# mit-han-lab/TinyChatEngine

Measured on NVIDIA H100. Metric: llama3_8b_awq_int4_batch1_decode_tokens_per_s, higher is better.
Workload: dtype w4a16 (int4 weights; activations fp16 -> 32-bit block fixed point = four int8 digit planes; int32 accumulate, fp32 scale)

## Files before the change

tinychatengine_b200/csrc/decode_persistent.cu:

```cuda
#include <stdio.h>

#include "persistent.h"
#include "w4a16_act_planes.cuh"

namespace tce {
namespace pk {

namespace {

TCE_DEVINL unsigned ld_acquire_gpu(const unsigned *p) {
    unsigned v;
    asm volatile("ld.acquire.gpu.global.u32 %0, [%1];" : "=r"(v) : "l"(p) : "memory");
    return v;
}
TCE_DEVINL void red_release_gpu(unsigned *p) { asm volatile("red.release.gpu.global.add.u32 [%0], 1;" ::"l"(p) : "memory"); }

TCE_DEVINL void st_ll(uint2 *p, uint32_t data, uint32_t tag, bool sys) {
    if (sys)
        asm volatile("st.relaxed.sys.global.v2.b32 [%0], {%1, %2};" ::"l"(p), "r"(data), "r"(tag) : "memory");
    else
        asm volatile("st.relaxed.gpu.global.v2.b32 [%0], {%1, %2};" ::"l"(p), "r"(data), "r"(tag) : "memory");
}
TCE_DEVINL uint4 ld_ll2(const uint2 *p, bool sys) {
    uint4 r;
// ... 109 lines not shown
    float *gx;
    int *gsum;
    float *red;
    float *rms;
    float *inv;
    float *rope;
    uint64_t *full, *empty, *red_full, *red_empty;
    uint64_t *rx;
    float *prx;
    uint64_t *prx_full;
    uint64_t *pfree;
    int2 *red_pos;
    uint32_t ring_u32, xs_u32, gx_u32, gsum_u32, full_u32, empty_u32, redfull_u32, redempty_u32;
    int nst;
};

__host__ __device__ inline int resid_floats(const Args &a) { return plane_ic(a.E / kW4Group); }

TCE_DEVINL PSmem carve(uint8_t *raw, const Args &a) {
    PSmem s;
    uint8_t *base = raw + ((1024u - (smem_u32(raw) & 1023u)) & 1023u);
    s.nst = a.nst;
    s.ring = base;
    uint8_t *p = base + (size_t)a.nst * kStageBytes;
    s.xs = p;
    p += a.xs_bytes;
    s.resid = reinterpret_cast<float *>(p);
    p += (size_t)resid_floats(a) * 4;
    s.gx = reinterpret_cast<float *>(p);
    p += (size_t)a.max_ng * 4;
    s.gsum = reinterpret_cast<int *>(p);
    p += (size_t)a.max_ng * 8;
    s.red = reinterpret_cast<float *>(p);
    p += (size_t)kRedBufs * kCW * 16 * 4;
    s.rms = reinterpret_cast<float *>(p);
    p += 32 * 4;
    s.inv = reinterpret_cast<float *>(p);
    p += kCW * 4;
    s.rope = reinterpret_cast<float *>(p);
    p += 256 * 4;
    s.prx = reinterpret_cast<float *>(p);
    p += kPairSlots * 16 * 4;
    s.full = reinterpret_cast<uint64_t *>(p);
    s.empty = s.full + a.nst;
    s.red_full = s.empty + a.nst;
    s.red_empty = s.red_full + kRedBufs;
    s.rx = s.red_empty + kRedBufs;
    s.prx_full = s.rx + 1;
    s.pfree = s.prx_full + kPairSlots;
    s.red_pos = reinterpret_cast<int2 *>(s.pfree + kPairSlots);
    s.ring_u32 = smem_u32(s.ring);
    s.xs_u32 = smem_u32(s.xs);
    s.gx_u32 = smem_u32(s.gx);
    s.gsum_u32 = smem_u32(s.gsum);
    s.full_u32 = smem_u32(s.full);
    s.empty_u32 = smem_u32(s.empty);
    s.redfull_u32 = smem_u32(s.red_full);
    s.redempty_u32 = smem_u32(s.red_empty);
    return s;
}

struct Ring {
    int stage = 0;
    uint32_t phase = 0;
    TCE_DEVINL void advance(int nst) {
        if (++stage == nst) {
            stage = 0;
            phase ^= 1;
        }
    }
};
struct Red {
    int rb = 0;
    uint32_t rphase = 0;
    TCE_DEVINL void advance() {
// ... 11 lines not shown
    t0 = (int)((T * (unsigned)cta) / (unsigned)ncta);
    t1 = (int)((T * (unsigned)(cta + 1)) / (unsigned)ncta);
}

struct AttnSplit {
    int kvh, split, ch0, ch1, nsplit;
};
TCE_DEVINL AttnSplit attn_split(int cta, int ncta, int KVH, int pos) {
    AttnSplit s;
    const int T = pos + 1;
    const int nch = (T + kKvChunk - 1) / kKvChunk;
    int NS = ncta / KVH;
    if (NS < 1) NS = 1;
    int cps = (nch + NS - 1) / NS;
    if (cps * 32 < nch) cps = (nch + 31) / 32;
    s.nsplit = (nch + cps - 1) / cps;
    s.kvh = cta / NS;
    s.split = cta - s.kvh * NS;
    if (s.kvh >= KVH || s.split >= s.nsplit) {
        s.ch0 = s.ch1 = 0;
        s.kvh = 0;
    } else {
        s.ch0 = s.split * cps;
        s.ch1 = min(nch, s.ch0 + cps);
    }
    return s;
}

TCE_DEVINL void produce_gemv(const GemvOp &op, const CUtensorMap *m0, const uint8_t *meta, const PSmem &sm, Ring &rs, int cta, int ncta, int rank,
                             uint32_t leader, uint64_t policy) {
    int t0, t1;
    partition(op, cta, ncta, t0, t1);
    const KRange kr = k_range(op.NG, rank);
    const uint32_t box_bytes = 16u * (uint32_t)kr.bw * 64u;
    const int nbox = (t1 - t0) * kr.nb;
    const uint8_t *rec = meta + (size_t)t0 * kr.nb * kBoxMetaBytes;
    int tile = t0, box = 0;
    for (int i = 0; i < nbox; i += 2) {
        const int n = min(2, nbox - i);
        mbar_wait(&sm.empty[rs.stage], rs.phase ^ 1);
        uint64_t *bar = &sm.full[rs.stage];
        uint8_t *dst = sm.ring + (size_t)rs.stage * kStageBytes;
        mbar_arrive_expect_tx_pred(bar, (uint32_t)n * (box_bytes + kBoxMetaBytes), leader);
#pragma unroll 1
        for (int b = 0; b < n; b++) {
            int row = op.gate_up ? tile * 8 : tile * 16;
            const CUtensorMap *m = m0;
            if (!op.gate_up && op.nseg > 1 && row >= op.rows0) {
                row -= op.rows0;
                m = m0 + 1;
                if (op.nseg > 2 && row >= op.rows1) {
                    row -= op.rows1;
                    m = m0 + 2;
                }
            }
            tma_load_3d_pred(dst + b * 16384, m, 0, row, box * kBoxGroups, bar, policy, leader);
            if (op.gate_up) tma_load_3d_pred(dst + b * 16384 + 8192, m + 1, 0, row, box * kBoxGroups, bar, policy, leader);
            if (++box == kr.nb) {
                box = 0;
                tile++;
            }
        }
        bulk_g2s_pred(dst + kMetaOff, rec + (size_t)i * kBoxMetaBytes, (uint32_t)n * kBoxMetaBytes, bar, policy, leader);
        __syncwarp();
        rs.advance(sm.nst);
    }
}

TCE_DEVINL void produce_attn(const Args &a, const LayerDesc &L, const CUtensorMap *kvmap, const PSmem &sm, Ring &rs, int cta, int ncta, int pos,
                             uint32_t leader, uint64_t policy) {
    const AttnSplit sp = attn_split(cta, ncta, a.KVH, pos);
    for (int c = sp.ch0; c < sp.ch1; c++) {
        mbar_wait(&sm.empty[rs.stage], rs.phase ^ 1);
        uint64_t *bar = &sm.full[rs.stage];
        uint8_t *dst = sm.ring + (size_t)rs.stage * kStageBytes;
        const int krow = L.k_row0 + sp.kvh * a.max_ctx + c * kKvChunk, vrow = L.v_row0 + sp.kvh * a.max_ctx + c * kKvChunk;
        mbar_arrive_expect_tx_pred(bar, 2u * kHalfBytes, leader);
        tma_load_2d_pred(dst, kvmap, 0, krow, bar, policy, leader);
        tma_load_2d_pred(dst + 8192, kvmap, 64, krow, bar, policy, leader);
        tma_load_2d_pred(dst + kHalfBytes, kvmap, 0, vrow, bar, policy, leader);
        tma_load_2d_pred(dst + kHalfBytes + 8192, kvmap, 64, vrow, bar, policy, leader);
        __syncwarp();
        rs.advance(sm.nst);
    }
}

TCE_DEVINL void producer_walk(const Args &a, const PSmem &sm, int cta, int ncta, int rank, int pos, int lane) {
    Ring rs;
    const uint64_t policy = l2_policy_evict_first();
    const uint32_t leader = (lane == 0) ? 1u : 0u;
    const int Lyr = a.num_layers, nphase = 5 * Lyr + 1;
    const CUtensorMap *wmaps = a.maps + (size_t)rank * (Lyr * 7 + 1);
    const CUtensorMap *kvmap = a.maps + (size_t)2 * (Lyr * 7 + 1);
#pragma unroll 1
    for (int p = 0; p < nphase; p++) {
        const int l = p / 5, k = p - 5 * l;
// ... 169 lines not shown
                const float4 r1 = *reinterpret_cast<const float4 *>(sm.resid + (size_t)ui * 8 + 4);
                x[0] = r0.x; x[1] = r0.y; x[2] = r0.z; x[3] = r0.w;
                x[4] = r1.x; x[5] = r1.y; x[6] = r1.z; x[7] = r1.w;
                if (a.tp_size == 1) {
                    uint4 w[4];
                    wait_ll2xN<4>(delta + (size_t)gu * 8, tag, false, w);
                    x[0] += __uint_as_float(w[0].x); x[1] += __uint_as_float(w[0].z); x[2] += __uint_as_float(w[1].x); x[3] += __uint_as_float(w[1].z);
                    x[4] += __uint_as_float(w[2].x); x[5] += __uint_as_float(w[2].z); x[6] += __uint_as_float(w[3].x); x[7] += __uint_as_float(w[3].z);
                } else {
                    tp_accumulate(x, delta + (size_t)gu * 8, a.tp_size, a.E, tag);
                }
            }
            *reinterpret_cast<float4 *>(sm.resid + (size_t)ui * 8) = make_float4(x[0], x[1], x[2], x[3]);
            *reinterpret_cast<float4 *>(sm.resid + (size_t)ui * 8 + 4) = make_float4(x[4], x[5], x[6], x[7]);
        }
        if (emit) {
#pragma unroll
            for (int i = 0; i < 8; i++) ss += x[i] * x[i];
            v[0] = x[0] * g0.x; v[1] = x[1] * g0.y; v[2] = x[2] * g0.z; v[3] = x[3] * g0.w;
            v[4] = x[4] * g1.x; v[5] = x[5] * g1.y; v[6] = x[6] * g1.z; v[7] = x[7] * g1.w;
            gemv::emit_unit<1>(sm.xs, xic, sm.gx, sm.gsum, ui, valid, v, lane);
        }
    }
    if (!emit) return;
    ss = warp_sum(ss);
    if (lane == 0) {
        sm.rms[pc.rank * kCW + cw] = ss;
        st_async_b32(pc.r_rms + (uint32_t)(pc.rank * kCW + cw) * 4u, __float_as_uint(ss), pc.r_bar);
    }
    named_bar_sync(1, kConsumerThreads);
}

struct UnitRegs {
    uint4 wa, wb, xe, xo;
    uint32_t z;
    uint32_t sc;
    int sxv;
};
TCE_DEVINL void unit_compute(const UnitRegs &u, uint32_t st_addr, float lscale, float &totA, float &totB) {
    constexpr uint32_t ML = 0x0f0f0f0fu, MH = 0xf0f0f0f0u;
    int accL[4], accH[4];
    mma_m16n8k32_u8s8_z(accL, u.wa.x & ML, u.wb.x & ML, u.wa.y & ML, u.wb.y & ML, u.xe.x, u.xe.y);
    mma_m16n8k32_u8s8_z(accH, u.wa.x & MH, u.wb.x & MH, u.wa.y & MH, u.wb.y & MH, u.xo.x, u.xo.y);
    mma_m16n8k32_u8s8(accL, u.wa.z & ML, u.wb.z & ML, u.wa.w & ML, u.wb.w & ML, u.xe.z, u.xe.w);
    mma_m16n8k32_u8s8(accH, u.wa.z & MH, u.wb.z & MH, u.wa.w & MH, u.wb.w & MH, u.xo.z, u.xo.w);
    const float2 sc = h2_to_f2(u.sc);
    const float st = lds_f32(st_addr) * lscale;
    const int zAq = (int)(u.z & 0xFFu), zBq = (int)(u.z >> 8);
    const int vA = (accL[0] << 8) + accL[1] + (((accH[0] << 8) + accH[1]) >> 4) - zAq * u.sxv;
    const int vB = (accL[2] << 8) + accL[3] + (((accH[2] << 8) + accH[3]) >> 4) - zBq * u.sxv;
    totA += (sc.x * st) * (float)vA;
    totB += (sc.y * st) * (float)vB;
}

TCE_DEVINL void hand_tile(const Args &a, const GemvOp &op, const PSmem &sm, Red &cs, float totA, float totB, int cw, int lane) {
    const int g = lane >> 2, t = lane & 3;
    float inv = sm.inv[cw];
    if (inv < 0.f) {
        mbar_wait_u32(smem_u32(sm.rx), inv < -1.5f ? 1u : 0u);
        inv = rms_inv(sm, op.IC, a.eps);
        __syncwarp();
        if (lane == 0) sm.inv[cw] = inv;
    }
    totA += __shfl_xor_sync(0xffffffffu, totA, 1);
    totB += __shfl_xor_sync(0xffffffffu, totB, 1);
    mbar_wait_u32(sm.redempty_u32 + (uint32_t)cs.rb * 8u, cs.rphase ^ 1);
    float *rbuf = sm.red + ((size_t)cs.rb * kCW + cw) * 16;
    if (t == 0) {
        rbuf[g] = totA * inv;
        rbuf[g + 8] = totB * inv;
    }
    __syncwarp();
    if (lane == 0) mbar_arrive_u32(sm.redfull_u32 + (uint32_t)cs.rb * 8u);
    cs.advance();
}

TCE_DEVINL void consume_gemv(const Args &a, const GemvOp &op, const PSmem &sm, Ring &rs, int rx_parity, int cta, int ncta, int rank, int cw, int p, int nphase) {
    int lane;
    asm volatile("mov.u32 %0, %%laneid;" : "=r"(lane));
    if (lane == 0) sm.inv[cw] = rx_parity >= 0 ? -1.f - (float)rx_parity : 1.f;
    __syncwarp();
    Red cs;
    {
        const int2 rp = sm.red_pos[cw];
        cs.rb = rp.x;
        cs.rphase = (uint32_t)rp.y;
    }
    const int g = lane >> 2, t = lane & 3;
    int t0, t1;
    partition(op, cta, ncta, t0, t1);
    const KRange kr = k_range(op.NG, rank);
    const int nb = kr.nb, nbox = (t1 - t0) * nb;
    const int lim = kr.ng - cw;
    const uint32_t w_lane = (uint32_t)cw * (op.gate_up ? 512u : 1024u) + (uint32_t)g * 64u + (uint32_t)t * 16u;
    const uint32_t wb_off = op.gate_up ? 8192u : 512u;
    const uint32_t m_lane = (uint32_t)kMetaOff + (uint32_t)(cw * 8 + g) * 4u;
    const uint32_t z_lane = (uint32_t)kMetaOff + 512u + (uint32_t)(cw * 8 + g) * 2u;
    const uint32_t x_lane = sm.xs_u32 + (uint32_t)((g >> 1) & 1) * (uint32_t)plane_ic(op.NG) * 2u + (uint32_t)(t * 2 + (g & 1)) * 16u + (uint32_t)cw * 256u;
    const uint32_t s_lane = sm.gsum_u32 + (uint32_t)(2 * cw + (t & 1)) * 4u;
    const uint32_t q_lane = sm.gx_u32 + (uint32_t)cw * 4u;
    const float lscale = (t == 0) ? 65536.f : (t == 1 ? 1.f : 0.f);
    const bool xl = g < 4;
    if (a.dbg && nbox > 0 && cw == 0 && lane == 0) {
        mbar_wait_u32(sm.full_u32 + (uint32_t)rs.stage * 8u, rs.phase);
        stamp(a, cta, nphase, p, 4);
    }
    int box = 0;
    float totA = 0.f, totB = 0.f;
    for (int left = nbox; left > 0; left -= 2) {
        const int box0 = box, box1 = (box0 + 1 == nb) ? 0 : box0 + 1;
        const bool two = left > 1;
        box = (box1 + 1 == nb) ? 0 : box1 + 1;
        const bool has0 = box0 * kBoxGroups < lim, has1 = two && box1 * kBoxGroups < lim;
        mbar_wait_u32(sm.full_u32 + (uint32_t)rs.stage * 8u, rs.phase);
        const uint32_t base = sm.ring_u32 + (uint32_t)rs.stage * (uint32_t)kStageBytes;
        const uint32_t wb_ = base + w_lane, mb_ = base + m_lane, zb_ = base + z_lane;
        UnitRegs u0, u1;
        u0.xe = u0.xo = u1.xe = u1.xo = make_uint4(0u, 0u, 0u, 0u);
        if (has0) {
            const uint32_t xb_ = x_lane + (uint32_t)box0 * 4096u;
            u0.wa = lds_u4(wb_);
            u0.wb = lds_u4(wb_ + wb_off);
            if (xl) {
                u0.xe = lds_u4(xb_);
                u0.xo = lds_u4(xb_ + 128u);
            }
            u0.sc = lds_u32(mb_);
            u0.z = lds_u16(zb_);
            u0.sxv = (int)lds_u32(s_lane + (uint32_t)box0 * 128u);
        }
        if (has1) {
            const uint32_t xb_ = x_lane + (uint32_t)box1 * 4096u;
            u1.wa = lds_u4(wb_ + 16384u);
            u1.wb = lds_u4(wb_ + 16384u + wb_off);
            if (xl) {
                u1.xe = lds_u4(xb_);
                u1.xo = lds_u4(xb_ + 128u);
            }
            u1.sc = lds_u32(mb_ + (uint32_t)kBoxMetaBytes);
            u1.z = lds_u16(zb_ + (uint32_t)kBoxMetaBytes);
            u1.sxv = (int)lds_u32(s_lane + (uint32_t)box1 * 128u);
        }
        if (has0) unit_compute(u0, q_lane + (uint32_t)box0 * 64u, lscale, totA, totB);
        const bool end0 = box0 + 1 == nb;
        float hA = 0.f, hB = 0.f;
        if (end0) {
            hA = totA;
            hB = totB;
            totA = totB = 0.f;
        }
        if (has1) unit_compute(u1, q_lane + (uint32_t)box1 * 64u, lscale, totA, totB);
        __syncwarp();
        if (lane == 0) mbar_arrive_u32(sm.empty_u32 + (uint32_t)rs.stage * 8u);
        rs.advance(sm.nst);
        if (left <= 2 && cw == 0 && lane == 0) stamp(a, cta, nphase, p, 5);
        const bool end1 = two && box1 + 1 == nb;
        if (end0) hand_tile(a, op, sm, cs, hA, hB, cw, lane);
        if (end1) {
            hand_tile(a, op, sm, cs, totA, totB, cw, lane);
            totA = totB = 0.f;
        }
    }
    __syncwarp();
    if (lane == 0) sm.red_pos[cw] = make_int2(cs.rb, (int)cs.rphase);
    __syncwarp();
    if (cw == 0 && lane == 0) stamp(a, cta, nphase, p, 6);
}

struct EpiState {
    unsigned long long best;
    uint32_t nsent, nrecv;
};

TCE_DEVINL void epilogue_gemv(const Args &a, const GemvOp &op, const PSmem &sm, Red &es, EpiState &st, uint2 *out_ll, int which, uint32_t tag, int cta, int ncta,
                              int p, int nphase) {
    int lane;
    asm volatile("mov.u32 %0, %%laneid;" : "=r"(lane));
    int t0, t1;
    partition(op, cta, ncta, t0, t1);
    const bool tp = a.tp_size > 1;
    const uint32_t rank = cluster_rank();
    const int tsplit = t0 + (t1 - t0 + 1) / 2;
    for (int tile = t0; tile < t1; tile++) {
        mbar_wait_u32(sm.redfull_u32 + (uint32_t)es.rb * 8u, es.rphase);
        if (tile == t1 - 1 && lane == 0) stamp(a, cta, nphase, p, 7);
        const float *rbuf = sm.red + (size_t)es.rb * kCW * 16;
        float v = 0.f;
        {
            const int row = lane & 15, w0 = (lane >> 4) * 8;
#pragma unroll
            for (int w = 0; w < 8; w++) v += rbuf[(w0 + w) * 16 + row];
        }
        v += __shfl_down_sync(0xffffffffu, v, 16);
        __syncwarp();
        if (lane == 0) mbar_arrive_u32(sm.redempty_u32 + (uint32_t)es.rb * 8u);
        es.advance();
        const bool mine = (tile >= tsplit) == (rank == 1u);
        const uint32_t slot = (mine ? st.nrecv : st.nsent) % kPairSlots;
        if (!mine) {
            const uint32_t n = st.nsent++;
            mbar_wait_cluster(smem_u32(sm.pfree + slot), ((n / kPairSlots) & 1u) ^ 1u);
            if (lane < 16)
                st_async_b32(map_to_cta(smem_u32(sm.prx + slot * 16 + lane), rank ^ 1u), __float_as_uint(v), map_to_cta(smem_u32(sm.prx_full + slot), rank ^ 1u));
            continue;
        }
        const uint32_t n = st.nrecv++;
        const uint32_t fb = smem_u32(sm.prx_full + slot);
        if (lane == 0) asm volatile("mbarrier.arrive.expect_tx.shared::cta.b64 _, [%0], %1;" ::"r"(fb), "r"(64u) : "memory");
        mbar_wait_u32(fb, (n / kPairSlots) & 1u);
        v += sm.prx[slot * 16 + (lane & 15)];
        __syncwarp();
        if (lane == 0) mbar_arrive_remote(map_to_cta(smem_u32(sm.pfree + slot), rank ^ 1u));
        switch (op.epi) {
            case PE_DELTA_LL:
                if (lane < 16) {
                    const size_t o = (size_t)a.tp_rank * a.E + (size_t)tile * 16 + lane;
                    if (tp) {
                        for (int pr = 0; pr < a.tp_size; pr++) st_ll(a.tp_delta[which][pr] + o, __float_as_uint(v), tag, true);
                    } else {
                        st_ll(out_ll + o, __float_as_uint(v), tag, false);
                    }
                }
                break;
            case PE_HALF_LL: {
                const float hi = __shfl_down_sync(0xffffffffu, v, 1);
                if (lane < 16 && !(lane & 1)) st_ll(out_ll + (size_t)tile * 8 + (lane >> 1), pack_half2(v, hi), tag, false);
                break;
            }
            case PE_SILU_LL: {
                const float up = __shfl_down_sync(0xffffffffu, v, 8);
                const float y = v / (1.f + __expf(-v)) * up;
                const float yhi = __shfl_down_sync(0xffffffffu, y, 1);
                if (lane < 8 && !(lane & 1)) st_ll(out_ll + (size_t)tile * 4 + (lane >> 1), pack_half2(y, yhi), tag, false);
                break;
            }
            case PE_LOGITS:
                if (lane < 16) {
                    const int idx = tile * 16 + lane;
                    a.logits[idx] = v;
                    const unsigned long long key = argmax_key(v, a.vocab_base + idx);
                    st.best = key > st.best ? key : st.best;
                }
                break;
        }
    }
}

TCE_DEVINL uint32_t kv_off(int r, int c) { return (uint32_t)((c >> 3) * 8192 + r * 128 + (((c & 7) ^ (r & 7)) << 4)); }

TCE_DEVINL float2 rope_pair(const uint2 *vec, int j, uint32_t tag, const float *cosr, const float *sinr) {
    const uint2 *pa = vec + j, *pb = vec + (j < 32 ? j + 32 : j - 32);
    uint2 wa = ld_ll1(pa, false), wb = ld_ll1(pb, false);
    if (wa.y != tag) wa.x = wait_ll1(pa, tag, false);
    if (wb.y != tag) wb.x = wait_ll1(pb, tag, false);
    const float2 x = h2_to_f2(wa.x), xp = h2_to_f2(wb.x);
    const float sgn = (j < 32) ? -1.f : 1.f;
    const int d = 2 * j;
    return make_float2(x.x * cosr[d] + sgn * xp.x * sinr[d], x.y * cosr[d + 1] + sgn * xp.y * sinr[d + 1]);
}

TCE_DEVINL void attention_phase(const Args &a, const LayerDesc &L, const PSmem &sm, Ring &rs, uint32_t tag_qkv, uint32_t tag_part, uint32_t tag_out, int cta,
                                int ncta, int pos, int ctid, int cw, int lane, int p, int nphase) {
    const AttnSplit sp = attn_split(cta, ncta, a.KVH, pos);
    const int nrep = a.nrep;
    const int g = lane >> 2, t = lane & 3;
    if (sp.ch0 < sp.ch1) {
        __half *sQ = reinterpret_cast<__half *>(sm.xs);
        float *sO = reinterpret_cast<float *>(sm.xs + 8 * 136 * 2);
        float *sML = sO + (size_t)kCW * nrep * 128;
        uint32_t *sKV = reinterpret_cast<uint32_t *>(sML + (size_t)kCW * nrep * 2);
        const float *cosr = sm.rope, *sinr = sm.rope + 128;
        const bool owns_new = sp.ch1 * kKvChunk > pos;
        static_assert(8 * 64 == kConsumerThreads, "one pass");
        {
            const int r = ctid >> 6, j = ctid & 63;
            float2 v = make_float2(0.f, 0.f);
// ... 304 lines not shown
    if (cta == 0 && ctid == 0) {
        const unsigned target = (epoch + 1u) * (unsigned)ncta;
        const long long t0 = clock64();
        while ((int)(ld_acquire_gpu(a.done) - target) < 0) {
            if (clock64() - t0 > kSpinLimit) __trap();
        }
        unsigned long long key = *reinterpret_cast<volatile unsigned long long *>(a.argmax_cell);
        if (a.tp_size > 1) {
            const uint32_t tag = tag_base + 2u * (uint32_t)nphase;
            for (int pr = 0; pr < a.tp_size; pr++) {
                st_ll(a.tp_keys[pr] + (size_t)a.tp_rank * 2, (uint32_t)(key >> 32), tag, true);
                st_ll(a.tp_keys[pr] + (size_t)a.tp_rank * 2 + 1, (uint32_t)key, tag, true);
            }
            key = 0ull;
            for (int pr = 0; pr < a.tp_size; pr++) {
                const uint32_t hi = wait_ll1(a.tp_keys[a.tp_rank] + (size_t)pr * 2, tag, true), lo = wait_ll1(a.tp_keys[a.tp_rank] + (size_t)pr * 2 + 1, tag, true);
                const unsigned long long k2 = ((unsigned long long)hi << 32) | lo;
                key = k2 > key ? k2 : key;
            }
        }
        *a.next_token = (int)(0xFFFFFFFFu - (unsigned)(key & 0xFFFFFFFFull));
        *a.argmax_cell = 0ull;
        *a.epoch = epoch + 1u;
    }
}

__global__ void repack_meta_kernel(W4Seg s0, W4Seg s1, W4Seg s2, int nseg, int gate_up, int g0, int ng, int nb, int zeros_w, int sf_w, int num_tiles, uint8_t *out) {
    const int idx = blockIdx.x * blockDim.x + threadIdx.x;
    if (idx >= num_tiles * nb * kBoxGroups) return;
    const int gi = idx % kBoxGroups, rb = idx / kBoxGroups;
    const int tile = rb / nb, box = rb - tile * nb;
    const int lg = kBoxGroups * box + gi, G = g0 + lg;
    uint8_t *rec = out + (size_t)rb * kBoxMetaBytes;
    __half *so = reinterpret_cast<__half *>(rec) + gi * 16;
    uint8_t *zo = rec + 512 + gi * 16;
    for (int r = 0; r < 16; r++) {
        const W4Seg *seg = &s0;
        int row;
        if (gate_up) {
            seg = (r < 8) ? &s0 : &s1;
            row = tile * 8 + (r & 7);
        } else {
            row = tile * 16 + r;
            if (nseg > 1 && row >= s0.rows) {
                row -= s0.rows;
                seg = &s1;
                if (nseg > 2 && row >= s1.rows) {
                    row -= s1.rows;
                    seg = &s2;
                }
            }
        }
        const int slot = (r & 7) * 2 + (r >> 3);
        if (lg < ng) {
            so[slot] = seg->scales[(size_t)row * sf_w + G];
            zo[slot] = (uint8_t)((seg->zeros[(size_t)row * zeros_w + (G >> 3)] >> ((G & 7) * 4)) & 0xFu);
        } else {
            so[slot] = __float2half(0.f);
            zo[slot] = 0;
        }
    }
}

}

int attn_scratch_bytes(int nrep) { return 8 * 136 * 2 + kCW * nrep * 128 * 4 + kCW * nrep * 2 * 4 + 2 * 64 * 4; }

int attn_nsplit_max(int ncta, int KVH, int max_ctx) {
    int NS = ncta / KVH;
    if (NS < 1) NS = 1;
    const int nch = (max_ctx + kKvChunk - 1) / kKvChunk;
    return NS < nch ? NS : nch;
}

static size_t fixed_bytes(const Args &a) {
    return (size_t)a.xs_bytes + (size_t)resid_floats(a) * 4 + (size_t)a.max_ng * 12 + (size_t)kRedBufs * kCW * 16 * 4 + 32 * 4 + kCW * 4 + 256 * 4 + (size_t)kPairSlots * 16 * 4 +
           (size_t)(2 * kMaxStages + 2 * kRedBufs + 1 + 2 * kPairSlots) * 8 + (size_t)kCW * 8 + 1024;
}
void plan_smem(Args &a, int smem_optin) {
    int xs = attn_scratch_bytes(a.nrep);
    for (int i = 0; i < OPI_COUNT; i++) xs = max(xs, 4 * plane_ic(a.op[i].NG));
    a.xs_bytes = (xs + 15) & ~15;
    a.nst = 0;
    const long long n = ((long long)smem_optin - (long long)fixed_bytes(a)) / kStageBytes;
    if (n >= 2) a.nst = (int)(n > kMaxStages ? kMaxStages : n);
}
size_t smem_bytes(const Args &a) { return fixed_bytes(a) + (size_t)a.nst * kStageBytes; }

cudaError_t repack_meta(Ctx *ctx, const W4Seg *segs, int nseg, int gate_up, int IC, const KRange &kr, uint8_t *out, cudaStream_t stream) {
    int rows = 0;
    for (int i = 0; i < nseg; i++) rows += segs[i].rows;
    const int num_tiles = rows / 16;
    const int zw = zeros_width(IC, kW4Group);
    const int total = num_tiles * kr.nb * kBoxGroups;
    if (total == 0) return cudaSuccess;
    repack_meta_kernel<<<(total + 127) / 128, 128, 0, stream>>>(segs[0], segs[nseg > 1 ? 1 : 0], segs[nseg > 2 ? 2 : 0], nseg, gate_up, kr.g0, kr.ng, kr.nb, zw, zw * 8,
                                                               num_tiles, out);
    (void)ctx;
    return cudaGetLastError();
}

cudaError_t encode_kv_tmap(CUtensorMap *out, const void *kv, long long rows) {
    const TmapEncodeFn fn = tmap_encoder();
    if (!fn) return cudaErrorNotSupported;
    const cuuint64_t gdim[2] = {128, (cuuint64_t)rows};
    const cuuint64_t gstride[1] = {256};
    const cuuint32_t box[2] = {64, (cuuint32_t)kKvChunk};
    const cuuint32_t estr[2] = {1, 1};
    const CUresult r = fn(out, CU_TENSOR_MAP_DATA_TYPE_UINT16, 2, const_cast<void *>(kv), gdim, gstride, box, estr, CU_TENSOR_MAP_INTERLEAVE_NONE,
                          CU_TENSOR_MAP_SWIZZLE_128B, CU_TENSOR_MAP_L2_PROMOTION_L2_256B, CU_TENSOR_MAP_FLOAT_OOB_FILL_NONE);
    return r == CUDA_SUCCESS ? cudaSuccess : cudaErrorInvalidValue;
}

static cudaLaunchConfig_t launch_config(Ctx *ctx, size_t smem, cudaStream_t stream, cudaLaunchAttribute *attr) {
    cudaLaunchConfig_t cfg = {};
    cfg.gridDim = dim3(ctx->num_sms);
    cfg.blockDim = dim3(kThreads);
    cfg.dynamicSmemBytes = smem;
    cfg.stream = stream;
    attr[0].id = cudaLaunchAttributeClusterDimension;
    attr[0].val.clusterDim.x = 2;
    attr[0].val.clusterDim.y = 1;
    attr[0].val.clusterDim.z = 1;
    cfg.attrs = attr;
    cfg.numAttrs = 1;
// ... 28 lines not shown
```

tinychatengine_b200/csrc/llama_decoder.cu:

```cuda
#include "llama_decoder.h"

#include "persistent.h"

#include <math.h>
#include <stdio.h>
#include <stdlib.h>
#include <string.h>

namespace tce {

#define DCK(call)                              \
    do {                                       \
        cudaError_t e__ = (call);              \
        if (e__ != cudaSuccess) return e__;    \
    } while (0)

static bool w4_ok(const tce_w4_tensor &t, int oc, int ic) { return t.w && t.zeros && t.scales && t.oc == oc && t.ic == ic; }

LlamaDecoder *LlamaDecoder::create(Ctx *ctx, int attn_chunk, const tce_llama_config &cfg, const tce_llama_weights &w, std::string *err) {
    auto bad = [&](const char *m) {
        *err = m;
        return (LlamaDecoder *)nullptr;
    };
    if (cfg.head_dim != 128) return bad("head_dim must be 128");
// ... 106 lines not shown
    *count = (int)bs_->gemv_ops.size();
    return cudaSuccess;
}

cudaError_t LlamaDecoder::tp_handle(void *out64) {
    if (tp_ <= 1 || !tp_buf_) return cudaErrorInvalidValue;
    static_assert(sizeof(cudaIpcMemHandle_t) == 64, "handle size");
    return cudaIpcGetMemHandle(reinterpret_cast<cudaIpcMemHandle_t *>(out64), tp_buf_.get());
}

cudaError_t LlamaDecoder::tp_connect(const void *handles, std::string *err) {
    if (tp_ <= 1) return cudaErrorInvalidValue;
    const cudaIpcMemHandle_t *h = reinterpret_cast<const cudaIpcMemHandle_t *>(handles);
    for (int p = 0; p < tp_; p++) {
        if (p == cfg_.tp_rank) {
            tp_peer_[p] = tp_buf_.get();
        } else {
            DCK(cudaIpcOpenMemHandle((void **)&tp_peer_[p], h[p], cudaIpcMemLazyEnablePeerAccess));
        }
    }
    DCK(build_persistent(err));
    tp_connected_ = true;
    return cudaSuccess;
}

cudaError_t LlamaDecoder::build_persistent(std::string *err) {
    const int E = cfg_.embed_dim, F = cfg_.hidden_dim, H = cfg_.num_heads, KVH = cfg_.num_kv_heads, hd = cfg_.head_dim, V = cfg_.vocab_size;
    const int Lyr = cfg_.num_layers, ncta = ctx_->num_sms;
    const int nrep = H / KVH;
    auto no = [&](const char *m) {
        if (err) *err = m;
        return cudaErrorNotSupported;
    };
    if (hd != 128 || nrep > 4 || ncta < KVH || F % 16 || V % 16) return no("shape outside the persistent kernel's envelope");
    if (ncta % 2) return no("odd SM count: the persistent kernel runs on clusters of two CTAs");
    pk::Args a{};
    auto mk = [&](int IC, int rows, int nseg, int gate_up, int rows0, int rows1, int x_mode, int epi) {
        pk::GemvOp o{};
        o.IC = IC;
        o.NG = IC / kW4Group;
        o.num_tiles = rows / 16;
        o.nseg = nseg;
        o.gate_up = gate_up;
        o.rows0 = rows0;
        o.rows1 = rows1;
        o.x_mode = x_mode;
        o.epi = epi;
        return o;
    };
    const bool tp = tp_ > 1;
    a.op[pk::OPI_QKV] = mk(E, (H + 2 * KVH) * hd, 3, 0, H * hd, KVH * hd, pk::PX_RMS_F32, pk::PE_HALF_LL);
    a.op[pk::OPI_O] = mk(H * hd, E, 1, 0, E, 0, pk::PX_HALF, pk::PE_DELTA_LL);
    a.op[pk::OPI_GATEUP] = mk(E, 2 * F, 2, 1, F, F, pk::PX_RMS_F32, pk::PE_SILU_LL);
    a.op[pk::OPI_DOWN] = mk(F, E, 1, 0, E, 0, pk::PX_HALF, pk::PE_DELTA_LL);
    a.op[pk::OPI_LMHEAD] = mk(E, V, 1, 0, V, 0, pk::PX_RMS_F32, pk::PE_LOGITS);
    int max_ng = 0, min_ng = 1 << 30;
    for (int i = 0; i < pk::OPI_COUNT; i++) {
        if (a.op[i].NG > max_ng) max_ng = a.op[i].NG;
        if (a.op[i].NG < min_ng) min_ng = a.op[i].NG;
        if (a.op[i].IC % kW4Group || a.op[i].num_tiles < 1) return no("bad GEMV shape");
    }
    if (min_ng < 2) return no("a GEMV with a single 128-group: nothing to split across a cluster of two CTAs");
    a.max_ng = (max_ng + 3) & ~3;
    a.E = E;
    a.nrep = nrep;
    pk::plan_smem(a, ctx_->smem_optin);
    if (a.nst < 2) return no("shared memory too small for the persistent kernel");
    if (!pk::pair_supported(ctx_, a)) return no("the device cannot co-schedule num_sms / 2 clusters of two CTAs");

    auto dalloc = [&](size_t bytes) -> void * {
        DevPtr<uint8_t> p;
        if (dev_alloc(p, bytes ? bytes : 16) != cudaSuccess) return nullptr;
        pk_allocs_.push_back(std::move(p));
        return pk_allocs_.back().get();
    };
    cudaStream_t s = ctx_->stream;
    const size_t nmaps = (size_t)Lyr * 7 + 1;
    std::vector<CUtensorMap> maps(2 * nmaps + 1);
    memset(maps.data(), 0, maps.size() * sizeof(CUtensorMap));
    std::vector<pk::LayerDesc> descs(Lyr);
    const size_t per_kv = (size_t)KVH * cfg_.max_ctx;
    for (int l = 0; l < Lyr; l++) {
        const tce_llama_layer &L = layers_[l];
        const tce_w4_tensor *t7[7] = {&L.q, &L.k, &L.v, &L.o, &L.gate, &L.up, &L.down};
        const int opi[7] = {pk::OPI_QKV, pk::OPI_QKV, pk::OPI_QKV, pk::OPI_O, pk::OPI_GATEUP, pk::OPI_GATEUP, pk::OPI_DOWN};
        for (int rank = 0; rank < 2; rank++) {
            for (int i = 0; i < 7; i++) {
                const pk::GemvOp &o = a.op[opi[i]];
                const pk::KRange kr = pk::k_range(o.NG, rank);
                DCK(encode_w4_tmap_units(&maps[rank * nmaps + (size_t)l * 7 + i], t7[i]->w, t7[i]->oc, t7[i]->ic, kr.bw, o.gate_up ? 8 : 16, kr.g0, kr.ng));
            }
        }
        pk::LayerDesc &D = descs[l];
        memset(&D, 0, sizeof(D));
        const W4Seg qkv[3] = {seg_of(L.q), seg_of(L.k), seg_of(L.v)}, o1[1] = {seg_of(L.o)}, gu[2] = {seg_of(L.gate), seg_of(L.up)}, d1[1] = {seg_of(L.down)};
        const W4Seg *segs[4] = {qkv, o1, gu, d1};
        const int nsegs[4] = {3, 1, 2, 1};
        const int ops4[4] = {pk::OPI_QKV, pk::OPI_O, pk::OPI_GATEUP, pk::OPI_DOWN};
        for (int rank = 0; rank < 2; rank++) {
            for (int i = 0; i < 4; i++) {
                const pk::GemvOp &o = a.op[ops4[i]];
                const pk::KRange kr = pk::k_range(o.NG, rank);
                uint8_t *m = (uint8_t *)dalloc((size_t)o.num_tiles * kr.nb * pk::kBoxMetaBytes);
                if (!m) return cudaErrorMemoryAllocation;
                DCK(pk::repack_meta(ctx_, segs[i], nsegs[i], o.gate_up, o.IC, kr, m, s));
                D.meta[rank][i] = m;
            }
        }
        D.input_norm = L.input_norm;
        D.post_norm = L.post_norm;
        D.k_cache = (__half *)kv_cache(l, 0);
        D.v_cache = (__half *)kv_cache(l, 1);
        D.k_row0 = (int)(((size_t)l * 2 + 0) * per_kv);
        D.v_row0 = (int)(((size_t)l * 2 + 1) * per_kv);
    }
    {
        const pk::GemvOp &o = a.op[pk::OPI_LMHEAD];
        const W4Seg lm[1] = {seg_of(w_.lm_head)};
        for (int rank = 0; rank < 2; rank++) {
            const pk::KRange kr = pk::k_range(o.NG, rank);
            DCK(encode_w4_tmap_units(&maps[rank * nmaps + (size_t)Lyr * 7], w_.lm_head.w, w_.lm_head.oc, w_.lm_head.ic, kr.bw, 16, kr.g0, kr.ng));
            uint8_t *m = (uint8_t *)dalloc((size_t)o.num_tiles * kr.nb * pk::kBoxMetaBytes);
            if (!m) return cudaErrorMemoryAllocation;
            DCK(pk::repack_meta(ctx_, lm, 1, 0, o.IC, kr, m, s));
            a.lm_meta[rank] = m;
        }
    }
    DCK(pk::encode_kv_tmap(&maps[2 * nmaps], d_kv_.get(), (long long)Lyr * 2 * per_kv));
    CUtensorMap *dmaps = (CUtensorMap *)dalloc(maps.size() * sizeof(CUtensorMap));
    pk::LayerDesc *ddesc = (pk::LayerDesc *)dalloc(descs.size() * sizeof(pk::LayerDesc));
    a.nsplit_max = pk::attn_nsplit_max(ncta, KVH, cfg_.max_ctx);
    const size_t n_qkv = (size_t)(H + 2 * KVH) * 64, n_attn = (size_t)H * 64, n_act = (size_t)F / 2, n_part = (size_t)H * a.nsplit_max * 130;
    const size_t ll_words = n_qkv + n_attn + n_act + n_part + (tp ? 0 : (size_t)2 * E);
    uint2 *ll = (uint2 *)dalloc(ll_words * sizeof(uint2));
    uint8_t *ctl = (uint8_t *)dalloc(32);
    if (!dmaps || !ddesc || !ll || !ctl) return cudaErrorMemoryAllocation;
    DCK(cudaMemcpyAsync(dmaps, maps.data(), maps.size() * sizeof(CUtensorMap), cudaMemcpyHostToDevice, s));
    DCK(cudaMemcpyAsync(ddesc, descs.data(), descs.size() * sizeof(pk::LayerDesc), cudaMemcpyHostToDevice, s));
    DCK(cudaMemsetAsync(ll, 0, ll_words * sizeof(uint2), s));
    DCK(cudaMemsetAsync(ctl, 0, 32, s));
    DCK(cudaStreamSynchronize(s));
    a.layers = ddesc;
    a.num_layers = Lyr;
    a.maps = dmaps;
    a.final_norm = w_.final_norm;
    a.embed = (const __half *)w_.embed_f16;
    a.embed_rows = V * tp_;
    a.qkv_ll = ll;
    a.attn_ll = a.qkv_ll + n_qkv;
    a.act_ll = a.attn_ll + n_attn;
    a.part_ll = a.act_ll + n_act;
    a.logits = io1_.logits.get();
    a.tokpos = io1_.req.get();
    a.next_token = io1_.next.get();
// ... 888 lines not shown
```

tinychatengine_b200/csrc/persistent.h:

```cpp
#pragma once
#include "kernels.h"

namespace tce {
namespace pk {

constexpr int kCW = 16;
constexpr int kAuxWarps = 4;
constexpr int kThreads = 32 * (kAuxWarps + kCW);
constexpr int kConsumerThreads = 32 * kCW;
constexpr int kHalfBytes = 16384;
constexpr int kBoxGroups = 16;
constexpr int kMetaOff = 2 * kHalfBytes;
constexpr int kBoxMetaBytes = 768;
constexpr int kStageBytes = 34816;
constexpr int kMaxStages = 6;
constexpr int kRedBufs = 3;
constexpr int kPairSlots = 8;
constexpr int kKvChunk = 64;

enum XMode : int { PX_HALF = 0, PX_RMS_F32 = 1 };
enum Epi : int { PE_HALF_LL = 0, PE_DELTA_LL = 1, PE_SILU_LL = 2, PE_LOGITS = 3 };
enum OpIdx : int { OPI_QKV = 0, OPI_O = 1, OPI_GATEUP = 2, OPI_DOWN = 3, OPI_LMHEAD = 4, OPI_COUNT = 5 };

struct GemvOp {
    int IC, NG;
    int num_tiles;
    int nseg, gate_up;
    int rows0, rows1;
    int x_mode, epi;
};

struct KRange {
    int g0, ng;
    int nb, bw;
};
__host__ __device__ inline KRange k_range(int NG, int rank) {
    KRange k;
    const int h = (NG + 1) / 2;
    k.g0 = rank ? h : 0;
    k.ng = rank ? NG - h : h;
    k.nb = (k.ng + kBoxGroups - 1) / kBoxGroups;
    k.bw = k.ng < kBoxGroups ? k.ng : kBoxGroups;
    return k;
}
__host__ __device__ inline int plane_ic(int NG) { return k_range(NG, 0).ng * 128; }

// ... 55 lines not shown
```

Baseline: 515.4.

## Widen GEMV output tile from 16 to 32 rows per box

Doubles the rows per weight tile so each TMA box carries 32 output rows and one stage holds one box instead of two 16-row boxes. Each consumer warp now issues four MMA chains sharing the same activation fragments, which reuses activation loads across more rows and halves the per-tile reduction and handoff overhead. The metadata record layout, repack kernel, tensor-map box heights, reduction buffers and epilogues are all resized so every lane now owns one row. In exchange there are fewer tiles, so work balance across CTAs gets coarser for small matrices, and each warp holds more registers.

```diff
diff --git a/tinychatengine_b200/csrc/decode_persistent.cu b/tinychatengine_b200/csrc/decode_persistent.cu
--- a/tinychatengine_b200/csrc/decode_persistent.cu
+++ b/tinychatengine_b200/csrc/decode_persistent.cu
@@ -165,7 +165,7 @@
     s.gsum = reinterpret_cast<int *>(p);
     p += (size_t)a.max_ng * 8;
     s.red = reinterpret_cast<float *>(p);
-    p += (size_t)kRedBufs * kCW * 16 * 4;
+    p += (size_t)kRedBufs * kCW * kTileRows * 4;
     s.rms = reinterpret_cast<float *>(p);
     p += 32 * 4;
     s.inv = reinterpret_cast<float *>(p);
@@ -173,7 +173,7 @@
     s.rope = reinterpret_cast<float *>(p);
     p += 256 * 4;
     s.prx = reinterpret_cast<float *>(p);
-    p += kPairSlots * 16 * 4;
+    p += kPairSlots * kTileRows * 4;
     s.full = reinterpret_cast<uint64_t *>(p);
     s.empty = s.full + a.nst;
     s.red_full = s.empty + a.nst;
@@ -251,36 +251,32 @@
     int t0, t1;
     partition(op, cta, ncta, t0, t1);
     const KRange kr = k_range(op.NG, rank);
-    const uint32_t box_bytes = 16u * (uint32_t)kr.bw * 64u;
+    const uint32_t stage_tx = (uint32_t)kTileRows * (uint32_t)kr.bw * 64u + (uint32_t)kBoxMetaBytes;
     const int nbox = (t1 - t0) * kr.nb;
     const uint8_t *rec = meta + (size_t)t0 * kr.nb * kBoxMetaBytes;
     int tile = t0, box = 0;
-    for (int i = 0; i < nbox; i += 2) {
-        const int n = min(2, nbox - i);
+    for (int i = 0; i < nbox; i++) {
         mbar_wait(&sm.empty[rs.stage], rs.phase ^ 1);
         uint64_t *bar = &sm.full[rs.stage];
         uint8_t *dst = sm.ring + (size_t)rs.stage * kStageBytes;
-        mbar_arrive_expect_tx_pred(bar, (uint32_t)n * (box_bytes + kBoxMetaBytes), leader);
-#pragma unroll 1
-        for (int b = 0; b < n; b++) {
-            int row = op.gate_up ? tile * 8 : tile * 16;
-            const CUtensorMap *m = m0;
-            if (!op.gate_up && op.nseg > 1 && row >= op.rows0) {
-                row -= op.rows0;
-                m = m0 + 1;
-                if (op.nseg > 2 && row >= op.rows1) {
-                    row -= op.rows1;
-                    m = m0 + 2;
-                }
-            }
-            tma_load_3d_pred(dst + b * 16384, m, 0, row, box * kBoxGroups, bar, policy, leader);
-            if (op.gate_up) tma_load_3d_pred(dst + b * 16384 + 8192, m + 1, 0, row, box * kBoxGroups, bar, policy, leader);
-            if (++box == kr.nb) {
-                box = 0;
-                tile++;
-            }
-        }
-        bulk_g2s_pred(dst + kMetaOff, rec + (size_t)i * kBoxMetaBytes, (uint32_t)n * kBoxMetaBytes, bar, policy, leader);
+        mbar_arrive_expect_tx_pred(bar, stage_tx, leader);
+        int row = op.gate_up ? tile * (kTileRows / 2) : tile * kTileRows;
+        const CUtensorMap *m = m0;
+        if (!op.gate_up && op.nseg > 1 && row >= op.rows0) {
+            row -= op.rows0;
+            m = m0 + 1;
+            if (op.nseg > 2 && row >= op.rows1) {
+                row -= op.rows1;
+                m = m0 + 2;
+            }
+        }
+        tma_load_3d_pred(dst, m, 0, row, box * kBoxGroups, bar, policy, leader);
+        if (op.gate_up) tma_load_3d_pred(dst + 16384, m + 1, 0, row, box * kBoxGroups, bar, policy, leader);
+        bulk_g2s_pred(dst + kMetaOff, rec + (size_t)i * kBoxMetaBytes, (uint32_t)kBoxMetaBytes, bar, policy, leader);
+        if (++box == kr.nb) {
+            box = 0;
+            tile++;
+        }
         __syncwarp();
         rs.advance(sm.nst);
     }
@@ -516,28 +512,39 @@
 }
 
 struct UnitRegs {
-    uint4 wa, wb, xe, xo;
+    uint4 wa, wb, wc, wd, xe, xo;
     uint32_t z;
-    uint32_t sc;
+    uint2 sc;
     int sxv;
 };
-TCE_DEVINL void unit_compute(const UnitRegs &u, uint32_t st_addr, float lscale, float &totA, float &totB) {
+struct RowSums {
+    float a, b, c, d;
+};
+TCE_DEVINL void unit_compute(const UnitRegs &u, uint32_t st_addr, float lscale, RowSums &tot) {
     constexpr uint32_t ML = 0x0f0f0f0fu, MH = 0xf0f0f0f0u;
-    int accL[4], accH[4];
+    int accL[4], accH[4], accL2[4], accH2[4];
     mma_m16n8k32_u8s8_z(accL, u.wa.x & ML, u.wb.x & ML, u.wa.y & ML, u.wb.y & ML, u.xe.x, u.xe.y);
     mma_m16n8k32_u8s8_z(accH, u.wa.x & MH, u.wb.x & MH, u.wa.y & MH, u.wb.y & MH, u.xo.x, u.xo.y);
+    mma_m16n8k32_u8s8_z(accL2, u.wc.x & ML, u.wd.x & ML, u.wc.y & ML, u.wd.y & ML, u.xe.x, u.xe.y);
+    mma_m16n8k32_u8s8_z(accH2, u.wc.x & MH, u.wd.x & MH, u.wc.y & MH, u.wd.y & MH, u.xo.x, u.xo.y);
     mma_m16n8k32_u8s8(accL, u.wa.z & ML, u.wb.z & ML, u.wa.w & ML, u.wb.w & ML, u.xe.z, u.xe.w);
     mma_m16n8k32_u8s8(accH, u.wa.z & MH, u.wb.z & MH, u.wa.w & MH, u.wb.w & MH, u.xo.z, u.xo.w);
-    const float2 sc = h2_to_f2(u.sc);
+    mma_m16n8k32_u8s8(accL2, u.wc.z & ML, u.wd.z & ML, u.wc.w & ML, u.wd.w & ML, u.xe.z, u.xe.w);
+    mma_m16n8k32_u8s8(accH2, u.wc.z & MH, u.wd.z & MH, u.wc.w & MH, u.wd.w & MH, u.xo.z, u.xo.w);
+    const float2 sc01 = h2_to_f2(u.sc.x), sc23 = h2_to_f2(u.sc.y);
     const float st = lds_f32(st_addr) * lscale;
-    const int zAq = (int)(u.z & 0xFFu), zBq = (int)(u.z >> 8);
-    const int vA = (accL[0] << 8) + accL[1] + (((accH[0] << 8) + accH[1]) >> 4) - zAq * u.sxv;
-    const int vB = (accL[2] << 8) + accL[3] + (((accH[2] << 8) + accH[3]) >> 4) - zBq * u.sxv;
-    totA += (sc.x * st) * (float)vA;
-    totB += (sc.y * st) * (float)vB;
-}
-
-TCE_DEVINL void hand_tile(const Args &a, const GemvOp &op, const PSmem &sm, Red &cs, float totA, float totB, int cw, int lane) {
+    const int z0 = (int)(u.z & 0xFFu), z1 = (int)((u.z >> 8) & 0xFFu), z2 = (int)((u.z >> 16) & 0xFFu), z3 = (int)(u.z >> 24);
+    const int v0 = (accL[0] << 8) + accL[1] + (((accH[0] << 8) + accH[1]) >> 4) - z0 * u.sxv;
+    const int v1 = (accL[2] << 8) + accL[3] + (((accH[2] << 8) + accH[3]) >> 4) - z1 * u.sxv;
+    const int v2 = (accL2[0] << 8) + accL2[1] + (((accH2[0] << 8) + accH2[1]) >> 4) - z2 * u.sxv;
+    const int v3 = (accL2[2] << 8) + accL2[3] + (((accH2[2] << 8) + accH2[3]) >> 4) - z3 * u.sxv;
+    tot.a += (sc01.x * st) * (float)v0;
+    tot.b += (sc01.y * st) * (float)v1;
+    tot.c += (sc23.x * st) * (float)v2;
+    tot.d += (sc23.y * st) * (float)v3;
+}
+
+TCE_DEVINL void hand_tile(const Args &a, const GemvOp &op, const PSmem &sm, Red &cs, RowSums tot, int cw, int lane) {
     const int g = lane >> 2, t = lane & 3;
     float inv = sm.inv[cw];
     if (inv < 0.f) {
@@ -546,13 +553,17 @@
         __syncwarp();
         if (lane == 0) sm.inv[cw] = inv;
     }
-    totA += __shfl_xor_sync(0xffffffffu, totA, 1);
-    totB += __shfl_xor_sync(0xffffffffu, totB, 1);
+    tot.a += __shfl_xor_sync(0xffffffffu, tot.a, 1);
+    tot.b += __shfl_xor_sync(0xffffffffu, tot.b, 1);
+    tot.c += __shfl_xor_sync(0xffffffffu, tot.c, 1);
+    tot.d += __shfl_xor_sync(0xffffffffu, tot.d, 1);
     mbar_wait_u32(sm.redempty_u32 + (uint32_t)cs.rb * 8u, cs.rphase ^ 1);
-    float *rbuf = sm.red + ((size_t)cs.rb * kCW + cw) * 16;
+    float *rbuf = sm.red + ((size_t)cs.rb * kCW + cw) * kTileRows;
     if (t == 0) {
-        rbuf[g] = totA * inv;
-        rbuf[g + 8] = totB * inv;
+        rbuf[g] = tot.a * inv;
+        rbuf[g + 8] = tot.b * inv;
+        rbuf[g + 16] = tot.c * inv;
+        rbuf[g + 24] = tot.d * inv;
     }
     __syncwarp();
     if (lane == 0) mbar_arrive_u32(sm.redfull_u32 + (uint32_t)cs.rb * 8u);
@@ -576,10 +587,10 @@
     const KRange kr = k_range(op.NG, rank);
     const int nb = kr.nb, nbox = (t1 - t0) * nb;
     const int lim = kr.ng - cw;
-    const uint32_t w_lane = (uint32_t)cw * (op.gate_up ? 512u : 1024u) + (uint32_t)g * 64u + (uint32_t)t * 16u;
-    const uint32_t wb_off = op.gate_up ? 8192u : 512u;
-    const uint32_t m_lane = (uint32_t)kMetaOff + (uint32_t)(cw * 8 + g) * 4u;
-    const uint32_t z_lane = (uint32_t)kMetaOff + 512u + (uint32_t)(cw * 8 + g) * 2u;
+    const uint32_t w_lane = (uint32_t)cw * (op.gate_up ? 1024u : 2048u) + (uint32_t)g * 64u + (uint32_t)t * 16u;
+    const uint32_t wc_off = op.gate_up ? 16384u : 1024u;
+    const uint32_t m_lane = (uint32_t)kMetaOff + (uint32_t)(cw * 8 + g) * 8u;
+    const uint32_t z_lane = (uint32_t)kMetaOff + 1024u + (uint32_t)(cw * 8 + g) * 4u;
     const uint32_t x_lane = sm.xs_u32 + (uint32_t)((g >> 1) & 1) * (uint32_t)plane_ic(op.NG) * 2u + (uint32_t)(t * 2 + (g & 1)) * 16u + (uint32_t)cw * 256u;
     const uint32_t s_lane = sm.gsum_u32 + (uint32_t)(2 * cw + (t & 1)) * 4u;
     const uint32_t q_lane = sm.gx_u32 + (uint32_t)cw * 4u;
@@ -590,59 +601,36 @@
         stamp(a, cta, nphase, p, 4);
     }
     int box = 0;
-    float totA = 0.f, totB = 0.f;
-    for (int left = nbox; left > 0; left -= 2) {
-        const int box0 = box, box1 = (box0 + 1 == nb) ? 0 : box0 + 1;
-        const bool two = left > 1;
-        box = (box1 + 1 == nb) ? 0 : box1 + 1;
-        const bool has0 = box0 * kBoxGroups < lim, has1 = two && box1 * kBoxGroups < lim;
+    RowSums tot = {0.f, 0.f, 0.f, 0.f};
+    for (int left = nbox; left > 0; left--) {
+        const bool has = box * kBoxGroups < lim;
         mbar_wait_u32(sm.full_u32 + (uint32_t)rs.stage * 8u, rs.phase);
-        const uint32_t base = sm.ring_u32 + (uint32_t)rs.stage * (uint32_t)kStageBytes;
-        const uint32_t wb_ = base + w_lane, mb_ = base + m_lane, zb_ = base + z_lane;
-        UnitRegs u0, u1;
-        u0.xe = u0.xo = u1.xe = u1.xo = make_uint4(0u, 0u, 0u, 0u);
-        if (has0) {
-            const uint32_t xb_ = x_lane + (uint32_t)box0 * 4096u;
-            u0.wa = lds_u4(wb_);
-            u0.wb = lds_u4(wb_ + wb_off);
+        if (has) {
+            const uint32_t base = sm.ring_u32 + (uint32_t)rs.stage * (uint32_t)kStageBytes;
+            const uint32_t wb_ = base + w_lane, xb_ = x_lane + (uint32_t)box * 4096u;
+            UnitRegs u;
+            u.wa = lds_u4(wb_);
+            u.wb = lds_u4(wb_ + 512u);
+            u.wc = lds_u4(wb_ + wc_off);
+            u.wd = lds_u4(wb_ + wc_off + 512u);
+            u.xe = u.xo = make_uint4(0u, 0u, 0u, 0u);
             if (xl) {
-                u0.xe = lds_u4(xb_);
-                u0.xo = lds_u4(xb_ + 128u);
-            }
-            u0.sc = lds_u32(mb_);
-            u0.z = lds_u16(zb_);
-            u0.sxv = (int)lds_u32(s_lane + (uint32_t)box0 * 128u);
-        }
-        if (has1) {
-            const uint32_t xb_ = x_lane + (uint32_t)box1 * 4096u;
-            u1.wa = lds_u4(wb_ + 16384u);
-            u1.wb = lds_u4(wb_ + 16384u + wb_off);
-            if (xl) {
-                u1.xe = lds_u4(xb_);
-                u1.xo = lds_u4(xb_ + 128u);
-            }
-            u1.sc = lds_u32(mb_ + (uint32_t)kBoxMetaBytes);
-            u1.z = lds_u16(zb_ + (uint32_t)kBoxMetaBytes);
-            u1.sxv = (int)lds_u32(s_lane + (uint32_t)box1 * 128u);
-        }
-        if (has0) unit_compute(u0, q_lane + (uint32_t)box0 * 64u, lscale, totA, totB);
-        const bool end0 = box0 + 1 == nb;
-        float hA = 0.f, hB = 0.f;
-        if (end0) {
-            hA = totA;
-            hB = totB;
-            totA = totB = 0.f;
-        }
-        if (has1) unit_compute(u1, q_lane + (uint32_t)box1 * 64u, lscale, totA, totB);
+                u.xe = lds_u4(xb_);
+                u.xo = lds_u4(xb_ + 128u);
+            }
+            u.sc = lds_u2(base + m_lane);
+            u.z = lds_u32(base + z_lane);
+            u.sxv = (int)lds_u32(s_lane + (uint32_t)box * 128u);
+            unit_compute(u, q_lane + (uint32_t)box * 64u, lscale, tot);
+        }
         __syncwarp();
         if (lane == 0) mbar_arrive_u32(sm.empty_u32 + (uint32_t)rs.stage * 8u);
         rs.advance(sm.nst);
-        if (left <= 2 && cw == 0 && lane == 0) stamp(a, cta, nphase, p, 5);
-        const bool end1 = two && box1 + 1 == nb;
-        if (end0) hand_tile(a, op, sm, cs, hA, hB, cw, lane);
-        if (end1) {
-            hand_tile(a, op, sm, cs, totA, totB, cw, lane);
-            totA = totB = 0.f;
+        if (left == 1 && cw == 0 && lane == 0) stamp(a, cta, nphase, p, 5);
+        if (++box == nb) {
+            box = 0;
+            hand_tile(a, op, sm, cs, tot, cw, lane);
+            tot.a = tot.b = tot.c = tot.d = 0.f;
         }
     }
     __syncwarp();
@@ -668,14 +656,10 @@
     for (int tile = t0; tile < t1; tile++) {
         mbar_wait_u32(sm.redfull_u32 + (uint32_t)es.rb * 8u, es.rphase);
         if (tile == t1 - 1 && lane == 0) stamp(a, cta, nphase, p, 7);
-        const float *rbuf = sm.red + (size_t)es.rb * kCW * 16;
+        const float *rbuf = sm.red + (size_t)es.rb * kCW * kTileRows;
         float v = 0.f;
-        {
-            const int row = lane & 15, w0 = (lane >> 4) * 8;
-#pragma unroll
-            for (int w = 0; w < 8; w++) v += rbuf[(w0 + w) * 16 + row];
-        }
-        v += __shfl_down_sync(0xffffffffu, v, 16);
+#pragma unroll
+        for (int w = 0; w < kCW; w++) v += rbuf[w * kTileRows + lane];
         __syncwarp();
         if (lane == 0) mbar_arrive_u32(sm.redempty_u32 + (uint32_t)es.rb * 8u);
         es.advance();
@@ -684,48 +668,45 @@
         if (!mine) {
             const uint32_t n = st.nsent++;
             mbar_wait_cluster(smem_u32(sm.pfree + slot), ((n / kPairSlots) & 1u) ^ 1u);
-            if (lane < 16)
-                st_async_b32(map_to_cta(smem_u32(sm.prx + slot * 16 + lane), rank ^ 1u), __float_as_uint(v), map_to_cta(smem_u32(sm.prx_full + slot), rank ^ 1u));
+            st_async_b32(map_to_cta(smem_u32(sm.prx + slot * kTileRows + lane), rank ^ 1u), __float_as_uint(v), map_to_cta(smem_u32(sm.prx_full + slot), rank ^ 1u));
             continue;
         }
         const uint32_t n = st.nrecv++;
         const uint32_t fb = smem_u32(sm.prx_full + slot);
-        if (lane == 0) asm volatile("mbarrier.arrive.expect_tx.shared::cta.b64 _, [%0], %1;" ::"r"(fb), "r"(64u) : "memory");
+        if (lane == 0) asm volatile("mbarrier.arrive.expect_tx.shared::cta.b64 _, [%0], %1;" ::"r"(fb), "r"((uint32_t)kTileRows * 4u) : "memory");
         mbar_wait_u32(fb, (n / kPairSlots) & 1u);
-        v += sm.prx[slot * 16 + (lane & 15)];
+        v += sm.prx[slot * kTileRows + lane];
         __syncwarp();
         if (lane == 0) mbar_arrive_remote(map_to_cta(smem_u32(sm.pfree + slot), rank ^ 1u));
         switch (op.epi) {
-            case PE_DELTA_LL:
-                if (lane < 16) {
-                    const size_t o = (size_t)a.tp_rank * a.E + (size_t)tile * 16 + lane;
-                    if (tp) {
-                        for (int pr = 0; pr < a.tp_size; pr++) st_ll(a.tp_delta[which][pr] + o, __float_as_uint(v), tag, true);
-                    } else {
-                        st_ll(out_ll + o, __float_as_uint(v), tag, false);
-                    }
+            case PE_DELTA_LL: {
+                const size_t o = (size_t)a.tp_rank * a.E + (size_t)tile * kTileRows + lane;
+                if (tp) {
+                    for (int pr = 0; pr < a.tp_size; pr++) st_ll(a.tp_delta[which][pr] + o, __float_as_uint(v), tag, true);
+                } else {
+                    st_ll(out_ll + o, __float_as_uint(v), tag, false);
                 }
                 break;
+            }
             case PE_HALF_LL: {
                 const float hi = __shfl_down_sync(0xffffffffu, v, 1);
-                if (lane < 16 && !(lane & 1)) st_ll(out_ll + (size_t)tile * 8 + (lane >> 1), pack_half2(v, hi), tag, false);
+                if (!(lane & 1)) st_ll(out_ll + (size_t)tile * (kTileRows / 2) + (lane >> 1), pack_half2(v, hi), tag, false);
                 break;
             }
             case PE_SILU_LL: {
-                const float up = __shfl_down_sync(0xffffffffu, v, 8);
+                const float up = __shfl_down_sync(0xffffffffu, v, 16);
                 const float y = v / (1.f + __expf(-v)) * up;
                 const float yhi = __shfl_down_sync(0xffffffffu, y, 1);
-                if (lane < 8 && !(lane & 1)) st_ll(out_ll + (size_t)tile * 4 + (lane >> 1), pack_half2(y, yhi), tag, false);
+                if (lane < 16 && !(lane & 1)) st_ll(out_ll + (size_t)tile * (kTileRows / 4) + (lane >> 1), pack_half2(y, yhi), tag, false);
                 break;
             }
-            case PE_LOGITS:
-                if (lane < 16) {
-                    const int idx = tile * 16 + lane;
-                    a.logits[idx] = v;
-                    const unsigned long long key = argmax_key(v, a.vocab_base + idx);
-                    st.best = key > st.best ? key : st.best;
-                }
+            case PE_LOGITS: {
+                const int idx = tile * kTileRows + lane;
+                a.logits[idx] = v;
+                const unsigned long long key = argmax_key(v, a.vocab_base + idx);
+                st.best = key > st.best ? key : st.best;
                 break;
+            }
         }
     }
 }
@@ -1096,16 +1077,16 @@
     const int tile = rb / nb, box = rb - tile * nb;
     const int lg = kBoxGroups * box + gi, G = g0 + lg;
     uint8_t *rec = out + (size_t)rb * kBoxMetaBytes;
-    __half *so = reinterpret_cast<__half *>(rec) + gi * 16;
-    uint8_t *zo = rec + 512 + gi * 16;
-    for (int r = 0; r < 16; r++) {
+    __half *so = reinterpret_cast<__half *>(rec) + gi * kTileRows;
+    uint8_t *zo = rec + 2 * kBoxGroups * kTileRows + gi * kTileRows;
+    for (int r = 0; r < kTileRows; r++) {
         const W4Seg *seg = &s0;
         int row;
         if (gate_up) {
-            seg = (r < 8) ? &s0 : &s1;
-            row = tile * 8 + (r & 7);
+            seg = (r < kTileRows / 2) ? &s0 : &s1;
+            row = tile * (kTileRows / 2) + (r & 15);
         } else {
-            row = tile * 16 + r;
+            row = tile * kTileRows + r;
             if (nseg > 1 && row >= s0.rows) {
                 row -= s0.rows;
                 seg = &s1;
@@ -1115,7 +1096,7 @@
                 }
             }
         }
-        const int slot = (r & 7) * 2 + (r >> 3);
+        const int slot = (r & 7) * 4 + (r >> 3);
         if (lg < ng) {
             so[slot] = seg->scales[(size_t)row * sf_w + G];
             zo[slot] = (uint8_t)((seg->zeros[(size_t)row * zeros_w + (G >> 3)] >> ((G & 7) * 4)) & 0xFu);
@@ -1138,7 +1119,8 @@
 }
 
 static size_t fixed_bytes(const Args &a) {
-    return (size_t)a.xs_bytes + (size_t)resid_floats(a) * 4 + (size_t)a.max_ng * 12 + (size_t)kRedBufs * kCW * 16 * 4 + 32 * 4 + kCW * 4 + 256 * 4 + (size_t)kPairSlots * 16 * 4 +
+    return (size_t)a.xs_bytes + (size_t)resid_floats(a) * 4 + (size_t)a.max_ng * 12 + (size_t)kRedBufs * kCW * kTileRows * 4 + 32 * 4 + kCW * 4 + 256 * 4 +
+           (size_t)kPairSlots * kTileRows * 4 +
            (size_t)(2 * kMaxStages + 2 * kRedBufs + 1 + 2 * kPairSlots) * 8 + (size_t)kCW * 8 + 1024;
 }
 void plan_smem(Args &a, int smem_optin) {
@@ -1154,7 +1136,7 @@
 cudaError_t repack_meta(Ctx *ctx, const W4Seg *segs, int nseg, int gate_up, int IC, const KRange &kr, uint8_t *out, cudaStream_t stream) {
     int rows = 0;
     for (int i = 0; i < nseg; i++) rows += segs[i].rows;
-    const int num_tiles = rows / 16;
+    const int num_tiles = rows / kTileRows;
     const int zw = zeros_width(IC, kW4Group);
     const int total = num_tiles * kr.nb * kBoxGroups;
     if (total == 0) return cudaSuccess;
diff --git a/tinychatengine_b200/csrc/llama_decoder.cu b/tinychatengine_b200/csrc/llama_decoder.cu
--- a/tinychatengine_b200/csrc/llama_decoder.cu
+++ b/tinychatengine_b200/csrc/llama_decoder.cu
@@ -162,14 +162,14 @@
         if (err) *err = m;
         return cudaErrorNotSupported;
     };
-    if (hd != 128 || nrep > 4 || ncta < KVH || F % 16 || V % 16) return no("shape outside the persistent kernel's envelope");
+    if (hd != 128 || nrep > 4 || ncta < KVH || F % pk::kTileRows || V % pk::kTileRows) return no("shape outside the persistent kernel's envelope");
     if (ncta % 2) return no("odd SM count: the persistent kernel runs on clusters of two CTAs");
     pk::Args a{};
     auto mk = [&](int IC, int rows, int nseg, int gate_up, int rows0, int rows1, int x_mode, int epi) {
         pk::GemvOp o{};
         o.IC = IC;
         o.NG = IC / kW4Group;
-        o.num_tiles = rows / 16;
+        o.num_tiles = rows / pk::kTileRows;
         o.nseg = nseg;
         o.gate_up = gate_up;
         o.rows0 = rows0;
@@ -218,7 +218,8 @@
             for (int i = 0; i < 7; i++) {
                 const pk::GemvOp &o = a.op[opi[i]];
                 const pk::KRange kr = pk::k_range(o.NG, rank);
-                DCK(encode_w4_tmap_units(&maps[rank * nmaps + (size_t)l * 7 + i], t7[i]->w, t7[i]->oc, t7[i]->ic, kr.bw, o.gate_up ? 8 : 16, kr.g0, kr.ng));
+                const int box_rows = o.gate_up ? pk::kTileRows / 2 : pk::kTileRows;
+                DCK(encode_w4_tmap_units(&maps[rank * nmaps + (size_t)l * 7 + i], t7[i]->w, t7[i]->oc, t7[i]->ic, kr.bw, box_rows, kr.g0, kr.ng));
             }
         }
         pk::LayerDesc &D = descs[l];
@@ -249,7 +250,7 @@
         const W4Seg lm[1] = {seg_of(w_.lm_head)};
         for (int rank = 0; rank < 2; rank++) {
             const pk::KRange kr = pk::k_range(o.NG, rank);
-            DCK(encode_w4_tmap_units(&maps[rank * nmaps + (size_t)Lyr * 7], w_.lm_head.w, w_.lm_head.oc, w_.lm_head.ic, kr.bw, 16, kr.g0, kr.ng));
+            DCK(encode_w4_tmap_units(&maps[rank * nmaps + (size_t)Lyr * 7], w_.lm_head.w, w_.lm_head.oc, w_.lm_head.ic, kr.bw, pk::kTileRows, kr.g0, kr.ng));
             uint8_t *m = (uint8_t *)dalloc((size_t)o.num_tiles * kr.nb * pk::kBoxMetaBytes);
             if (!m) return cudaErrorMemoryAllocation;
             DCK(pk::repack_meta(ctx_, lm, 1, 0, o.IC, kr, m, s));
diff --git a/tinychatengine_b200/csrc/persistent.h b/tinychatengine_b200/csrc/persistent.h
--- a/tinychatengine_b200/csrc/persistent.h
+++ b/tinychatengine_b200/csrc/persistent.h
@@ -9,9 +9,10 @@
 constexpr int kThreads = 32 * (kAuxWarps + kCW);
 constexpr int kConsumerThreads = 32 * kCW;
 constexpr int kHalfBytes = 16384;
+constexpr int kTileRows = 32;
 constexpr int kBoxGroups = 16;
 constexpr int kMetaOff = 2 * kHalfBytes;
-constexpr int kBoxMetaBytes = 768;
+constexpr int kBoxMetaBytes = 1536;
 constexpr int kStageBytes = 34816;
 constexpr int kMaxStages = 6;
 constexpr int kRedBufs = 3;
```

Result: faster. 540.0, median of 6 (+4.8%).
